# OwshenNetwork/owshen

Hardware: NVIDIA H100
Metric: groth16_withdraw_proofs_per_sec (higher is better)
Workload: dtype u256 (8x32-bit Montgomery limbs, integer)

## Files before the change

owshen_b200/csrc/common.cuh:

```cuda
#pragma once
#include <cuda_runtime.h>
#include <stdint.h>
#include <stdio.h>
#include <string.h>
#include <vector>
#include "../../include/owshen_b200.h"
#include "fp.cuh"
#include "ec.cuh"

namespace og {

constexpr int N_SLOTS = 64;
constexpr int MAX_LANES = 2;

struct NttTables;

}

struct og_ctx {
    int device = 0;
    int sm_count = 132;
    cudaStream_t stream = nullptr;
    cudaStream_t main_stream = nullptr;
    cudaStream_t lane_hi[og::MAX_LANES] = {nullptr}, lane_lo[og::MAX_LANES] = {nullptr};
    cudaEvent_t lane_ev[og::MAX_LANES] = {nullptr}, fork_ev = nullptr;
    cudaStream_t acc_stream = nullptr;
    cudaEvent_t acc_ev = nullptr;
    int lane = 0;
    cudaEvent_t ev0 = nullptr, ev1 = nullptr;
    uint64_t launches = 0;
    char err[512] = {0};
    void* slot_ptr[og::N_SLOTS] = {nullptr};
    size_t slot_cap[og::N_SLOTS] = {0};
    int* d_flag = nullptr;
    int* h_flag = nullptr;
    og::NttTables* ntt[32] = {nullptr};
    void* g1_fixed = nullptr;
    void* g2_fixed = nullptr;
    void* bjj_fixed = nullptr;
    bool digits_smem_opt_in = false;

    bool prof_on = false;
    struct ProfRec { const char* name; cudaEvent_t a, b; };
    std::vector<ProfRec> prof;
    std::vector<cudaEvent_t> ev_pool;
    cudaEvent_t prof_event();

    void* slot(int id, size_t bytes);
};

namespace og {

#define OG_CUDA(ctx, call)                                                                        \
    do {                                                                                          \
        cudaError_t e_ = (call);                                                                  \
        if (e_ != cudaSuccess) {                                                                  \
            snprintf((ctx)->err, sizeof((ctx)->err), "%s:%d: %s: %s", __FILE__, __LINE__, #call,  \
                     cudaGetErrorString(e_));                                                     \
            return OG_E_CUDA;                                                                     \
        }                                                                                         \
    } while (0)

#define OG_TRY(expr)                  \
    do {                              \
        int32_t rc_ = (expr);         \
        if (rc_ != OG_OK) return rc_; \
    } while (0)

#define OG_LAUNCHN(ctx, name, kernel, grid, block, smem, ...)                                     \
    do {                                                                                          \
        cudaEvent_t pa_ = nullptr, pb_ = nullptr;                                                 \
        if ((ctx)->prof_on) { pa_ = (ctx)->prof_event(); pb_ = (ctx)->prof_event();               \
                              cudaEventRecord(pa_, (ctx)->stream); }                              \
        kernel<<<(grid), (block), (smem), (ctx)->stream>>>(__VA_ARGS__);                          \
        if (pa_) { cudaEventRecord(pb_, (ctx)->stream); (ctx)->prof.push_back({(name), pa_, pb_}); } \
        (ctx)->launches++;                                                                        \
        OG_CUDA(ctx, cudaGetLastError());                                                         \
    } while (0)
#define OG_LAUNCH(ctx, kernel, grid, block, smem, ...) OG_LAUNCHN(ctx, #kernel, kernel, grid, block, smem, __VA_ARGS__)

#define OG_SLOT(ctx, var, type, id, bytes)                       \
    type* var = (type*)(ctx)->slot((id), (bytes));               \
    if (!var) return OG_E_NOMEM

enum Slot {
    S_IO_A = 0, S_IO_B, S_IO_C, S_IO_D, S_IO_E, S_IO_F, S_IO_G, S_IO_H,
    S_MSM_POINTS, S_MSM_SCALARS, S_MSM_COUNTS, S_MSM_OFFSETS, S_MSM_CURSOR, S_MSM_SORTED, S_MSM_BUCKETS,
    S_MSM_SEG, S_MSM_OUT, S_MSM_HEAVY, S_MSM_MISC,
    S_NTT_DATA,
    S_PR_WIT, S_PR_ABC, S_PR_SCALARS, S_PR_SORTED, S_PR_COUNTS, S_PR_OFFSETS, S_PR_CURSOR, S_PR_BUCKETS,
    S_PR_SEG, S_PR_SUMS, S_PR_OUT, S_PR_PUB, S_PR_MISC, S_PR_HEAVY,
    S_SETUP_A, S_SETUP_B, S_SETUP_C,
    S_L1_ABC, S_L1_SCALARS, S_L1_SORTED, S_L1_COUNTS, S_L1_OFFSETS, S_L1_CURSOR, S_L1_BUCKETS, S_L1_SEG, S_L1_HEAVY, S_L1_MSM_MISC,
    S_PR_AFF, S_L1_AFF, S_MSM_AFF,
    S_COUNT
};
static_assert(S_COUNT <= N_SLOTS, "grow N_SLOTS");

static inline cudaError_t stream_handoff(cudaEvent_t ev, cudaStream_t from, cudaStream_t to) {
    cudaError_t e = cudaEventRecord(ev, from);
    return e != cudaSuccess ? e : cudaStreamWaitEvent(to, ev, 0);
}

static inline bool aligned32(const void* p) { return (((uintptr_t)p) & 31) == 0; }

int32_t check_flag(og_ctx* ctx);
int32_t clear_flag(og_ctx* ctx);

template <class F>
__device__ __forceinline__ F load_canonical(const uint8_t* p, int* flag) {
    const uint32_t* q = reinterpret_cast<const uint32_t*>(p);
    uint32_t c[8];
#pragma unroll
    for (int i = 0; i < 8; i++) c[i] = q[i];
    if (!F::canonical_lt_mod(c)) { atomicOr(flag, 1); for (int i = 0; i < 8; i++) c[i] = 0; }
    return F::from_canonical(c);
}
template <class F>
__device__ __forceinline__ void store_canonical(uint8_t* p, const F& v) {
    uint32_t c[8];
    v.to_canonical(c);
    uint32_t* q = reinterpret_cast<uint32_t*>(p);
#pragma unroll
    for (int i = 0; i < 8; i++) q[i] = c[i];
}

template <class F>
static inline bool host_load(F& out, const uint8_t* p) {
    uint32_t c[8];
    memcpy(c, p, 32);
    if (!F::canonical_lt_mod(c)) return false;
    out = F::from_canonical(c);
    return true;
}
template <class F>
static inline void host_store(uint8_t* p, const F& v) {
    uint32_t c[8];
    v.to_canonical(c);
    memcpy(p, c, 32);
}

int32_t mimc_init(og_ctx* ctx);
void mimc_constants_host(Fr* out91);

}
```

owshen_b200/csrc/groth16.cu:

```cuda
#include "groth16.cuh"
#include "mimc.cuh"
#include "msm.cuh"
#include "ntt.cuh"
#include "withdraw_circuit.hpp"
#include <stdlib.h>

namespace og {

__global__ void __launch_bounds__(128) k_extras(const uint8_t* __restrict__ rs, uint32_t batch, uint32_t n_vars, uint32_t w_stride,
                                                Fr* __restrict__ W, Fr* __restrict__ rs_m, int* flag) {
    uint32_t p = blockIdx.x * blockDim.x + threadIdx.x;
    if (p >= batch) return;
    Fr r = load_canonical<Fr>(rs + 64ull * p, flag);
    Fr s = load_canonical<Fr>(rs + 64ull * p + 32, flag);
    Fr* w = W + (size_t)p * w_stride;
    w[n_vars] = Fr::one();
    w[n_vars + 1] = r;
    rs_m[2 * p] = r;
    rs_m[2 * p + 1] = s;
}

__global__ void __launch_bounds__(128) k_witness_in(const uint8_t* __restrict__ in, uint32_t batch, uint32_t n_vars, uint32_t w_stride,
                                                    Fr* __restrict__ W, int* flag) {
    uint64_t t = (uint64_t)blockIdx.x * blockDim.x + threadIdx.x;
// ... 220 lines not shown
    memcpy(hC.data() + 64ull * (n_priv + pk->n_supp + m), beta1, 64);

    int32_t rc = OG_OK;
    auto fail = [&](int32_t code) { pk_free(pk); return code; };
    if ((rc = clear_flag(ctx)) != OG_OK) return fail(rc);
    {
        uint8_t* stage;
        if ((rc = upload(ctx, &stage, hA.data(), hA.size())) != OG_OK) return fail(rc);
        if (cudaMalloc(&pk->tabA, sizeof(G1Affine) * (size_t)pk->nA * pk->n_windows[0]) != cudaSuccess) { cudaFree(stage); return fail(OG_E_NOMEM); }
        rc = g1_bytes_to_mont(ctx, stage, pk->nA, pk->tabA);
        if (rc == OG_OK) rc = msm_build_table_g1(ctx, pk->tabA, pk->nA, pk->c[0], pk->n_windows[0]);
        cudaStreamSynchronize(ctx->stream); cudaFree(stage);
        if (rc != OG_OK) return fail(rc);
    }
    {
        uint8_t* stage;
        if ((rc = upload(ctx, &stage, hC.data(), hC.size())) != OG_OK) return fail(rc);
        if (cudaMalloc(&pk->tabC, sizeof(G1Affine) * (size_t)pk->nC * pk->n_windows[2]) != cudaSuccess) { cudaFree(stage); return fail(OG_E_NOMEM); }
        rc = g1_bytes_to_mont(ctx, stage, pk->nC, pk->tabC);
        if (rc == OG_OK) rc = msm_build_table_g1(ctx, pk->tabC, pk->nC, pk->c[2], pk->n_windows[2]);
        cudaStreamSynchronize(ctx->stream); cudaFree(stage);
        if (rc != OG_OK) return fail(rc);
    }
    {
        uint8_t* stage;
        if ((rc = upload(ctx, &stage, hB.data(), hB.size())) != OG_OK) return fail(rc);
        if (cudaMalloc(&pk->tabB, sizeof(G2Affine) * (size_t)pk->nB * pk->n_windows[1]) != cudaSuccess) { cudaFree(stage); return fail(OG_E_NOMEM); }
        rc = g2_bytes_to_mont(ctx, stage, pk->nB, pk->tabB);
        if (rc == OG_OK) rc = msm_build_table_g2(ctx, pk->tabB, pk->nB, pk->c[1], pk->n_windows[1]);
        cudaStreamSynchronize(ctx->stream); cudaFree(stage);
        if (rc != OG_OK) return fail(rc);
    }
    if ((rc = upload(ctx, &pk->supp, supp.data(), 4ull * supp.size())) != OG_OK) return fail(rc);
    cudaStreamSynchronize(ctx->stream);
    if ((rc = upload_csr(ctx, rd, pk->n_constraints, nv, &pk->a_ptr, &pk->a_col, &pk->a_val)) != OG_OK) return fail(rc);
    if ((rc = upload_csr(ctx, rd, pk->n_constraints, nv, &pk->b_ptr, &pk->b_col, &pk->b_val)) != OG_OK) return fail(rc);
    if ((rc = check_flag(ctx)) != OG_OK) return fail(rc);
    *out = pk;
    return OG_OK;
}

bool pk_on_device_of(const og_pk* pk, const og_ctx* ctx) { return pk && ctx && pk->device == ctx->device; }

void pk_info(const og_pk* pk, uint32_t* n_vars, uint32_t* n_pub, uint32_t* log_m, uint32_t* depth) {
    if (n_vars) *n_vars = pk->n_vars;
    if (n_pub) *n_pub = pk->n_pub;
    if (log_m) *log_m = pk->log_m;
    if (depth) *depth = pk->depth;
}

struct ChunkBufs {
    Fr *W, *rs_m, *abc, *ntt_tmp, *bsc, *csc;
    uint32_t *counts, *offsets, *cursor, *sorted, *heavy;
    G1XYZZ *bk1, *lvl1, *totA, *totC;
    G2XYZZ *bk2, *lvl2, *totB;
    void *aff1, *aff2;
    uint32_t w_stride, bsc_stride, csc_stride;
};

#ifdef OG_EXPERIMENT_AFFINE
static uint32_t affine_mode() { return env_u32("OG_AFFINE", 0); }
#else
static uint32_t affine_mode() { return 0; }
#endif

static int32_t alloc_chunk(og_ctx* ctx, const og_pk* pk, uint32_t batch, uint32_t B, int lane, ChunkBufs& b) {
    const uint32_t m = 1u << pk->log_m;
    b.w_stride = pk->n_vars + 2;
    b.bsc_stride = pk->nB;
    b.csc_stride = pk->nC;
    size_t max_pts = pk->nC > pk->nA ? pk->nC : pk->nA;
    size_t n_keys = (size_t)B * pk->max_nb;
    auto S = [&](int id0, int id1) { return lane ? id1 : id0; };
    b.W = (Fr*)ctx->slot(S_PR_WIT, sizeof(Fr) * (size_t)batch * b.w_stride);
    b.rs_m = (Fr*)ctx->slot(S_PR_MISC, sizeof(Fr) * 2 * (size_t)batch);
    b.abc = (Fr*)ctx->slot(S(S_PR_ABC, S_L1_ABC), sizeof(Fr) * (size_t)B * 3 * m * 2);
    b.bsc = (Fr*)ctx->slot(S(S_PR_SCALARS, S_L1_SCALARS), sizeof(Fr) * (size_t)B * (b.bsc_stride + b.csc_stride));
    b.sorted = (uint32_t*)ctx->slot(S(S_PR_SORTED, S_L1_SORTED), 4 * (size_t)B * max_pts * pk->max_windows);
    b.counts = (uint32_t*)ctx->slot(S(S_PR_COUNTS, S_L1_COUNTS), 4 * n_keys);
    b.offsets = (uint32_t*)ctx->slot(S(S_PR_OFFSETS, S_L1_OFFSETS), 4 * (n_keys + 1));
    b.cursor = (uint32_t*)ctx->slot(S(S_PR_CURSOR, S_L1_CURSOR), 4 * n_keys);
    b.heavy = (uint32_t*)ctx->slot(S(S_PR_HEAVY, S_L1_HEAVY), 4 * (2 * n_keys + 4));
    b.bk2 = (G2XYZZ*)ctx->slot(S(S_PR_BUCKETS, S_L1_BUCKETS), sizeof(G2XYZZ) * n_keys);
    b.lvl2 = (G2XYZZ*)ctx->slot(S(S_PR_SEG, S_L1_SEG), sizeof(G2XYZZ) * msm_lvl_elems(B, pk->max_nb));
    b.totA = (G1XYZZ*)ctx->slot(S_PR_SUMS, (sizeof(G1XYZZ) * 2 + sizeof(G2XYZZ)) * (size_t)batch);
    if (!b.W || !b.rs_m || !b.abc || !b.bsc || !b.sorted || !b.counts || !b.offsets || !b.cursor || !b.heavy || !b.bk2 || !b.lvl2 || !b.totA)
        return OG_E_NOMEM;
    b.aff1 = b.aff2 = nullptr;
    if (affine_mode()) {
        size_t need = 0;
        if (affine_mode() & 1) need = msm_aff_scratch_bytes_g1(n_keys);
        if ((affine_mode() & 2) && msm_aff_scratch_bytes_g2((size_t)B * pk->nb[1]) > need) need = msm_aff_scratch_bytes_g2((size_t)B * pk->nb[1]);
        void* a = ctx->slot(S(S_PR_AFF, S_L1_AFF), need);
        if (!a) return OG_E_NOMEM;
        if (affine_mode() & 1) b.aff1 = a;
        if (affine_mode() & 2) b.aff2 = a;
    }
    b.ntt_tmp = b.abc + (size_t)B * 3 * m;
    b.csc = b.bsc + (size_t)B * b.bsc_stride;
    b.bk1 = reinterpret_cast<G1XYZZ*>(b.bk2);
    b.lvl1 = reinterpret_cast<G1XYZZ*>(b.lvl2);
    b.totC = b.totA + batch;
    b.totB = reinterpret_cast<G2XYZZ*>(b.totC + batch);
    return OG_OK;
}

static int32_t run_msm_g1(og_ctx* ctx, const og_pk* pk, int which, ChunkBufs& b, uint32_t B, const G1Affine* table, uint32_t n_pts,
                          const Fr* scalars, uint32_t stride, G1XYZZ* totals) {
    DigitPlan plan;
    plan.scalars = reinterpret_cast<const uint32_t*>(scalars);
    plan.n = n_pts; plan.scalar_stride = stride; plan.n_problems = B;
    plan.c = pk->c[which]; plan.n_windows = pk->n_windows[which]; plan.nb = pk->nb[which];
    plan.key_stride_problem = 1; plan.key_stride_window = 0; plan.tidx_window_stride = n_pts;
    plan.montgomery = 1;
    uint32_t n_keys = B * pk->nb[which];
    OG_TRY(msm_sort_digits(ctx, plan, n_keys, b.counts, b.offsets, b.cursor, b.sorted));
    return msm_buckets_g1(ctx, table, b.sorted, b.offsets, b.counts, B, pk->nb[which], (uint64_t)B * n_pts * pk->n_windows[which], b.bk1, b.lvl1, b.heavy, b.cursor, totals, b.aff1);
}
static int32_t run_msm_g2(og_ctx* ctx, const og_pk* pk, int which, ChunkBufs& b, uint32_t B, const G2Affine* table, uint32_t n_pts,
                          const Fr* scalars, uint32_t stride, G2XYZZ* totals) {
    DigitPlan plan;
    plan.scalars = reinterpret_cast<const uint32_t*>(scalars);
    plan.n = n_pts; plan.scalar_stride = stride; plan.n_problems = B;
    plan.c = pk->c[which]; plan.n_windows = pk->n_windows[which]; plan.nb = pk->nb[which];
    plan.key_stride_problem = 1; plan.key_stride_window = 0; plan.tidx_window_stride = n_pts;
    plan.montgomery = 1;
    uint32_t n_keys = B * pk->nb[which];
    OG_TRY(msm_sort_digits(ctx, plan, n_keys, b.counts, b.offsets, b.cursor, b.sorted));
    return msm_buckets_g2(ctx, table, b.sorted, b.offsets, b.counts, B, pk->nb[which], (uint64_t)B * n_pts * pk->n_windows[which], b.bk2, b.lvl2, b.heavy, b.cursor, totals, b.aff2);
}

struct WitnessSource {
    const uint8_t *d_null = nullptr, *d_sec = nullptr, *d_rec = nullptr, *d_sib = nullptr;
    const uint32_t* d_bits = nullptr;
    const uint8_t* d_wit = nullptr;
    uint8_t* d_public = nullptr;
};

static int32_t prove_chunk(og_ctx* ctx, const og_pk* pk, ChunkBufs& b, const WitnessSource& src, uint32_t off, uint32_t B,
                           const uint8_t* d_rs, uint8_t* d_proofs) {
    const uint32_t m = 1u << pk->log_m, n_priv = pk->n_vars - pk->n_pub - 1;
    Fr* W = b.W + (size_t)off * b.w_stride;
    Fr* rs_m = b.rs_m + 2 * (size_t)off;
    if (src.d_wit) {
        uint64_t tot = (uint64_t)B * pk->n_vars;
        OG_LAUNCH(ctx, k_witness_in, (unsigned)((tot + 127) / 128), 128, 0, src.d_wit + 32ull * off * pk->n_vars, B, pk->n_vars, b.w_stride, W, ctx->d_flag);
    } else {
        WithdrawLayout L = WithdrawLayout::make(pk->depth);
        OG_TRY(withdraw_witness_strided_dev(ctx, L, b.w_stride, src.d_null + 32ull * off, src.d_sec + 32ull * off, src.d_rec + 32ull * off,
                                            src.d_sib + 32ull * off * pk->depth, src.d_bits + off, B, W));
        if (src.d_public) OG_LAUNCH(ctx, k_public_out, (B * pk->n_pub + 127) / 128, 128, 0, W, b.w_stride, B, pk->n_pub, src.d_public + 32ull * off * pk->n_pub);
    }
    OG_LAUNCH(ctx, k_extras, (B + 127) / 128, 128, 0, d_rs + 64ull * off, B, pk->n_vars, b.w_stride, W, rs_m, ctx->d_flag);
    CsrDev A{pk->a_ptr, pk->a_col, pk->a_val}, Bm{pk->b_ptr, pk->b_col, pk->b_val};
    OG_LAUNCH(ctx, k_abc, dim3((m + 127) / 128, B), 128, 0, A, Bm, pk->n_constraints, pk->n_pub, pk->log_m, W, b.w_stride, B, b.abc);
    OG_TRY(ntt_mont_dev(ctx, b.abc, b.ntt_tmp, pk->log_m, 3 * B, 1, 0, 1));
    OG_TRY(ntt_mont_dev(ctx, b.abc, b.ntt_tmp, pk->log_m, 3 * B, 0, 1, 2));
    uint32_t mx = n_priv > pk->n_supp ? n_priv : pk->n_supp;
    OG_LAUNCH(ctx, k_compose, dim3((mx + 127) / 128, B), 128, 0, W, b.w_stride, rs_m, pk->supp, pk->n_supp, pk->n_vars, pk->n_pub, m,
              b.bsc, b.bsc_stride, b.csc, b.csc_stride);
    OG_LAUNCH(ctx, k_pointwise, dim3((m + 127) / 128, B), 128, 0, b.abc, pk->log_m, B, b.csc, b.csc_stride, n_priv + pk->n_supp);
    OG_TRY(run_msm_g1(ctx, pk, 0, b, B, pk->tabA, pk->nA, W, b.w_stride, b.totA + off));
    OG_TRY(run_msm_g1(ctx, pk, 2, b, B, pk->tabC, pk->nC, b.csc, b.csc_stride, b.totC + off));
    OG_TRY(run_msm_g2(ctx, pk, 1, b, B, pk->tabB, pk->nB, b.bsc, b.bsc_stride, b.totB + off));
    OG_LAUNCH(ctx, k_assemble_g1, (B + 31) / 32, 32, 0, b.totA + off, b.totC + off, rs_m, B, d_proofs + 256ull * off);
    OG_LAUNCH(ctx, k_assemble_g2, (B + 31) / 32, 32, 0, b.totB + off, B, d_proofs + 256ull * off);
    return OG_OK;
}

static uint32_t chunk_limit(const og_pk* pk) {
    uint64_t max_pts = pk->nC > pk->nA ? pk->nC : pk->nA;
    uint64_t by_entries = 0xF0000000ull / (max_pts * pk->max_windows);
    uint64_t by_keys = 0x7FFFFFFFull / pk->max_nb;
    uint64_t lim = by_entries < by_keys ? by_entries : by_keys;
    return (uint32_t)(lim < 1 ? 1 : lim);
}

static uint32_t chunk_size(const og_pk* pk, uint32_t batch) {
    uint32_t c = env_u32("OG_CHUNK", 1024);
    if (c > chunk_limit(pk)) c = chunk_limit(pk);
    return c < batch ? c : batch;
// ... 77 lines not shown
```

owshen_b200/csrc/msm.cu:

```cuda
#include "msm.cuh"
#include "glv.cuh"
#include <stdlib.h>
#if !defined(OG_MSM_G1) && !defined(OG_MSM_G2)
#error "compile msm.cu with -DOG_MSM_G1 or -DOG_MSM_G2"
#endif

namespace og {

template <class F> struct FieldIO;
template <> struct FieldIO<Fq> {
    static constexpr int BYTES = 32;
    static __device__ __forceinline__ Fq load(const uint8_t* p, int* flag) { return load_canonical<Fq>(p, flag); }
    static __device__ __forceinline__ void store(uint8_t* p, const Fq& v) { store_canonical(p, v); }
};
template <> struct FieldIO<Fq2> {
    static constexpr int BYTES = 64;
    static __device__ __forceinline__ Fq2 load(const uint8_t* p, int* flag) {
        return Fq2{load_canonical<Fq>(p, flag), load_canonical<Fq>(p + 32, flag)};
    }
    static __device__ __forceinline__ void store(uint8_t* p, const Fq2& v) { store_canonical(p, v.c0); store_canonical(p + 32, v.c1); }
};

template <class F>
__global__ void __launch_bounds__(128) k_points_to_mont(const uint8_t* __restrict__ in, uint64_t n, Affine<F>* __restrict__ out, int* flag) {
// ... 10 lines not shown
    constexpr int B = FieldIO<F>::BYTES;
    Affine<F> p = in[i];
    FieldIO<F>::store(out + 2 * B * i, p.x);
    FieldIO<F>::store(out + 2 * B * i + B, p.y);
}

#ifdef OG_MSM_G1
int32_t g1_bytes_to_mont(og_ctx* ctx, const uint8_t* d_in, uint64_t n, G1Affine* d_out) {
    if (n) OG_LAUNCH(ctx, k_points_to_mont<Fq>, (unsigned)((n + 127) / 128), 128, 0, d_in, n, d_out, ctx->d_flag);
    return OG_OK;
}
#endif

#ifdef OG_MSM_G2
int32_t g2_bytes_to_mont(og_ctx* ctx, const uint8_t* d_in, uint64_t n, G2Affine* d_out) {
    if (n) OG_LAUNCH(ctx, k_points_to_mont<Fq2>, (unsigned)((n + 127) / 128), 128, 0, d_in, n, d_out, ctx->d_flag);
    return OG_OK;
}
#endif

#ifdef OG_MSM_G1
int32_t g1_mont_to_bytes(og_ctx* ctx, const G1Affine* d_in, uint64_t n, uint8_t* d_out) {
    if (n) OG_LAUNCH(ctx, k_points_from_mont<Fq>, (unsigned)((n + 127) / 128), 128, 0, d_in, n, d_out);
    return OG_OK;
}
#endif

#ifdef OG_MSM_G2
int32_t g2_mont_to_bytes(og_ctx* ctx, const G2Affine* d_in, uint64_t n, uint8_t* d_out) {
    if (n) OG_LAUNCH(ctx, k_points_from_mont<Fq2>, (unsigned)((n + 127) / 128), 128, 0, d_in, n, d_out);
    return OG_OK;
}
#endif


#ifdef OG_MSM_G1
struct DigitIter {
    uint32_t s[9];
    __device__ __forceinline__ bool load(const DigitPlan& P, uint32_t prob, uint64_t i, int* flag) {
        const uint32_t* sp = P.scalars + ((uint64_t)prob * P.scalar_stride + i) * 8;
        if (P.montgomery) {
            Fr v;
#pragma unroll
            for (int j = 0; j < 8; j++) v.l[j] = sp[j];
            v.to_canonical(s);
        } else {
#pragma unroll
            for (int j = 0; j < 8; j++) s[j] = sp[j];
            if (!Fr::canonical_lt_mod(s)) { atomicOr(flag, 1); return false; }
        }
        s[8] = 0;
        return (s[0] | s[1] | s[2] | s[3] | s[4] | s[5] | s[6] | s[7]) != 0;
    }
    template <class Fn>
    __device__ __forceinline__ void for_each(const DigitPlan& P, Fn f) const {
        const uint32_t c = P.c, half = 1u << (c - 1), mask = (1u << c) - 1;
        uint32_t carry = 0;
        for (uint32_t w = 0; w < P.n_windows; w++) {
            uint32_t bit = w * c, word = bit >> 5, sh = bit & 31;
            uint64_t two = ((uint64_t)s[word + 1] << 32) | s[word];
            uint32_t v = ((uint32_t)(two >> sh) & mask) + carry;
            uint32_t neg = v > half;
            uint32_t mag = neg ? (1u << c) - v : v;
            carry = neg;
            if (mag) f(w, mag - 1, neg);
        }
    }
};

template <bool SCATTER>
__global__ void __launch_bounds__(256) k_digits(DigitPlan P, uint32_t* __restrict__ counts, const uint32_t* __restrict__ offsets,
                                                uint32_t* __restrict__ cursor, uint32_t* __restrict__ sorted, int* flag) {
    uint64_t i = (uint64_t)blockIdx.x * blockDim.x + threadIdx.x;
    uint32_t prob = blockIdx.y;
    if (i >= P.n) return;
    DigitIter it;
    if (!it.load(P, prob, i, flag)) return;
    it.for_each(P, [&](uint32_t w, uint32_t b, uint32_t neg) {
        uint32_t key = (prob * P.key_stride_problem + w * P.key_stride_window) * P.nb + b;
        if (!SCATTER) {
            atomicAdd(&counts[key], 1u);
        } else {
            uint32_t pos = atomicAdd(&cursor[key], 1u);
            sorted[pos] = (((uint32_t)i + w * P.tidx_window_stride) << 1) | neg;
        }
    });
}

constexpr uint32_t DIG_TILE = 4096, DIG_THREADS = 256, DIG_MAX_NB_COUNT = 32768;

__global__ void __launch_bounds__(DIG_THREADS) k_digits_count_tiled(DigitPlan P, uint32_t* __restrict__ counts, int* flag) {
    extern __shared__ uint32_t hist[];
    const uint32_t prob = blockIdx.y, nb = P.nb;
    const uint64_t lo = (uint64_t)blockIdx.x * DIG_TILE;
    const uint64_t hi = lo + DIG_TILE < P.n ? lo + DIG_TILE : P.n;
    const uint32_t key0 = prob * P.key_stride_problem * nb;
    for (uint32_t b = threadIdx.x; b < nb; b += DIG_THREADS) hist[b] = 0;
    __syncthreads();
    for (uint64_t i = lo + threadIdx.x; i < hi; i += DIG_THREADS) {
        DigitIter it;
        if (it.load(P, prob, i, flag)) it.for_each(P, [&](uint32_t, uint32_t b, uint32_t) { atomicAdd(&hist[b], 1u); });
    }
    __syncthreads();
    for (uint32_t b = threadIdx.x; b < nb; b += DIG_THREADS) if (hist[b]) atomicAdd(&counts[key0 + b], hist[b]);
}

constexpr uint32_t SCAN_THREADS = 256, SCAN_PER_THREAD = 8, SCAN_TILE = SCAN_THREADS * SCAN_PER_THREAD;

__device__ __forceinline__ uint32_t block_exclusive_scan(uint32_t v, uint32_t* total) {
    __shared__ uint32_t warp_sums[SCAN_THREADS / 32];
    __shared__ uint32_t block_total;
    uint32_t lane = threadIdx.x & 31, wid = threadIdx.x >> 5;
    uint32_t inc = v;
#pragma unroll
    for (int d = 1; d < 32; d <<= 1) { uint32_t t = __shfl_up_sync(0xffffffffu, inc, d); if (lane >= (uint32_t)d) inc += t; }
    if (lane == 31) warp_sums[wid] = inc;
    __syncthreads();
    if (wid == 0) {
        uint32_t w = lane < SCAN_THREADS / 32 ? warp_sums[lane] : 0, winc = w;
#pragma unroll
        for (int d = 1; d < 8; d <<= 1) { uint32_t t = __shfl_up_sync(0xffffffffu, winc, d); if (lane >= (uint32_t)d) winc += t; }
        if (lane < SCAN_THREADS / 32) warp_sums[lane] = winc - w;
        if (lane == SCAN_THREADS / 32 - 1) block_total = winc;
    }
    __syncthreads();
    uint32_t r = inc - v + warp_sums[wid];
    *total = block_total;
    __syncthreads();
    return r;
}

__global__ void __launch_bounds__(SCAN_THREADS) k_scan_tiles(const uint32_t* __restrict__ counts, uint32_t n, uint32_t* __restrict__ tile_sums) {
    uint32_t base = blockIdx.x * SCAN_TILE + threadIdx.x * SCAN_PER_THREAD, s = 0;
#pragma unroll
    for (uint32_t k = 0; k < SCAN_PER_THREAD; k++) if (base + k < n) s += counts[base + k];
    uint32_t total;
    block_exclusive_scan(s, &total);
    if (threadIdx.x == 0) tile_sums[blockIdx.x] = total;
}
__global__ void __launch_bounds__(SCAN_THREADS) k_scan_tile_sums(uint32_t* __restrict__ tile_sums, uint32_t n_tiles, uint32_t* __restrict__ grand_total) {
    uint32_t run = 0;
    for (uint32_t base = 0; base < n_tiles; base += SCAN_THREADS) {
        uint32_t i = base + threadIdx.x;
        uint32_t v = i < n_tiles ? tile_sums[i] : 0, total;
        uint32_t ex = block_exclusive_scan(v, &total);
        if (i < n_tiles) tile_sums[i] = run + ex;
        run += total;
    }
    if (threadIdx.x == 0) *grand_total = run;
}
__global__ void __launch_bounds__(SCAN_THREADS) k_scan_apply(const uint32_t* __restrict__ counts, uint32_t n, const uint32_t* __restrict__ tile_sums,
                                                            uint32_t* __restrict__ offsets, uint32_t* __restrict__ cursor) {
    uint32_t base = blockIdx.x * SCAN_TILE + threadIdx.x * SCAN_PER_THREAD;
    uint32_t c[SCAN_PER_THREAD], s = 0;
#pragma unroll
    for (uint32_t k = 0; k < SCAN_PER_THREAD; k++) { c[k] = base + k < n ? counts[base + k] : 0; s += c[k]; }
    uint32_t total;
    uint32_t run = tile_sums[blockIdx.x] + block_exclusive_scan(s, &total);
#pragma unroll
    for (uint32_t k = 0; k < SCAN_PER_THREAD; k++) {
        if (base + k < n) { offsets[base + k] = run; cursor[base + k] = run; }
        run += c[k];
    }
}

int32_t msm_sort_digits(og_ctx* ctx, const DigitPlan& plan, uint32_t n_keys, uint32_t* d_counts, uint32_t* d_offsets,
                        uint32_t* d_cursor, uint32_t* d_sorted) {
    OG_CUDA(ctx, cudaMemsetAsync(d_counts, 0, sizeof(uint32_t) * (size_t)n_keys, ctx->stream));
    if (plan.n == 0 || plan.n_problems == 0) {
        OG_CUDA(ctx, cudaMemsetAsync(d_offsets, 0, sizeof(uint32_t) * ((size_t)n_keys + 1), ctx->stream));
        return OG_OK;
    }
    const bool tiled = plan.key_stride_window == 0 && plan.nb <= DIG_MAX_NB_COUNT;
    if (tiled && !ctx->digits_smem_opt_in) {
        OG_CUDA(ctx, cudaFuncSetAttribute(k_digits_count_tiled, cudaFuncAttributeMaxDynamicSharedMemorySize, (int)(4 * DIG_MAX_NB_COUNT)));
        ctx->digits_smem_opt_in = true;
    }
    dim3 grid((unsigned)((plan.n + 255) / 256), plan.n_problems);
    dim3 tgrid((unsigned)((plan.n + DIG_TILE - 1) / DIG_TILE), plan.n_problems);
    if (tiled) OG_LAUNCH(ctx, k_digits_count_tiled, tgrid, DIG_THREADS, 4 * (size_t)plan.nb, plan, d_counts, ctx->d_flag);
    else OG_LAUNCHN(ctx, "k_digits_count", k_digits<false>, grid, 256, 0, plan, d_counts, nullptr, nullptr, nullptr, ctx->d_flag);
    {
        uint32_t n_tiles = (n_keys + SCAN_TILE - 1) / SCAN_TILE;
        OG_SLOT(ctx, tile_sums, uint32_t, ctx->lane ? S_L1_MSM_MISC : S_MSM_MISC, 4 * (size_t)n_tiles);
        OG_LAUNCH(ctx, k_scan_tiles, n_tiles, SCAN_THREADS, 0, d_counts, n_keys, tile_sums);
        OG_LAUNCH(ctx, k_scan_tile_sums, 1, SCAN_THREADS, 0, tile_sums, n_tiles, d_offsets + n_keys);
        OG_LAUNCH(ctx, k_scan_apply, n_tiles, SCAN_THREADS, 0, d_counts, n_keys, tile_sums, d_offsets, d_cursor);
    }
    OG_LAUNCHN(ctx, "k_digits_scatter", k_digits<true>, grid, 256, 0, plan, d_counts, d_offsets, d_cursor, d_sorted, ctx->d_flag);
    return OG_OK;
}
#endif


constexpr uint32_t ORDER_BINS = 2048;
template <class F>
__global__ void __launch_bounds__(1024) k_bucket_order(const uint32_t* __restrict__ counts, uint32_t nb, uint32_t* __restrict__ perm) {
    __shared__ uint32_t hist[ORDER_BINS];
    const uint32_t g = blockIdx.x, t = threadIdx.x;
    const uint32_t* c = counts + (size_t)g * nb;
    for (uint32_t i = t; i < ORDER_BINS; i += 1024) hist[i] = 0;
    __syncthreads();
    for (uint32_t b = t; b < nb; b += 1024) atomicAdd(&hist[ORDER_BINS - 1 - min(c[b], ORDER_BINS - 1)], 1u);
    __syncthreads();
    __shared__ uint32_t pair[1024];
    uint32_t a0 = hist[2 * t], a1 = hist[2 * t + 1];
    pair[t] = a0 + a1;
    __syncthreads();
    for (uint32_t d = 1; d < 1024; d <<= 1) {
        uint32_t v = t >= d ? pair[t - d] : 0;
        __syncthreads();
        pair[t] += v;
        __syncthreads();
    }
    uint32_t base = t ? pair[t - 1] : 0;
    hist[2 * t] = base;
    hist[2 * t + 1] = base + a0;
    __syncthreads();
    for (uint32_t b = t; b < nb; b += 1024) {
        uint32_t pos = atomicAdd(&hist[ORDER_BINS - 1 - min(c[b], ORDER_BINS - 1)], 1u);
        perm[(size_t)g * nb + pos] = g * nb + b;
    }
}

template <class F>
__device__ __forceinline__ Affine<F> fetch_point(const Affine<F>* __restrict__ table, uint32_t e) {
    Affine<F> p = table[e >> 1];
    if (e & 1) p.y = p.y.neg();
    return p;
}

#ifdef OG_MSM_G1
struct SmAcc1 {
    uint4* base;
    __device__ __forceinline__ Fq ld(int coord) const {
        Fq v;
        uint4 a = base[(coord * 2 + 0) * 128], b = base[(coord * 2 + 1) * 128];
        v.l[0] = a.x; v.l[1] = a.y; v.l[2] = a.z; v.l[3] = a.w; v.l[4] = b.x; v.l[5] = b.y; v.l[6] = b.z; v.l[7] = b.w;
        return v;
    }
    __device__ __forceinline__ void st(int coord, const Fq& v) const {
// ... 818 lines not shown
```

owshen_b200/csrc/msm.cuh:

```cuda
#pragma once
#include "common.cuh"

namespace og {

struct DigitPlan {
    const uint32_t* scalars;
    uint64_t n;
    uint64_t scalar_stride;
    uint32_t n_problems;
    uint32_t c, n_windows, nb;
    uint32_t key_stride_problem, key_stride_window;
    uint32_t tidx_window_stride;
    int32_t montgomery;
};

static inline uint32_t msm_windows(uint32_t c) { return (255 + c - 1) / c; }

int32_t msm_sort_digits(og_ctx* ctx, const DigitPlan& plan, uint32_t n_keys, uint32_t* d_counts,
                        uint32_t* d_offsets , uint32_t* d_cursor, uint32_t* d_sorted);

int32_t msm_buckets_g1(og_ctx* ctx, const G1Affine* d_table, const uint32_t* d_sorted, const uint32_t* d_offsets,
                       const uint32_t* d_counts, uint32_t n_groups, uint32_t nb, uint64_t n_entries_max, G1XYZZ* d_buckets,
                       G1XYZZ* d_lvl, uint32_t* d_heavy, uint32_t* d_perm, G1XYZZ* d_totals, void* aff_scratch = nullptr);
int32_t msm_buckets_g2(og_ctx* ctx, const G2Affine* d_table, const uint32_t* d_sorted, const uint32_t* d_offsets,
                       const uint32_t* d_counts, uint32_t n_groups, uint32_t nb, uint64_t n_entries_max, G2XYZZ* d_buckets,
                       G2XYZZ* d_lvl, uint32_t* d_heavy, uint32_t* d_perm, G2XYZZ* d_totals, void* aff_scratch = nullptr);
size_t msm_aff_scratch_bytes_g1(uint64_t n_keys);
size_t msm_aff_scratch_bytes_g2(uint64_t n_keys);
static inline size_t msm_lvl_elems(uint32_t n_groups, uint32_t nb) { return 4 * ((size_t)n_groups * ((nb + 7) / 8) + 16); }

int32_t msm_g1_dev(og_ctx* ctx, const uint8_t* d_points, const uint8_t* d_scalars, uint64_t n, uint8_t* d_out64);
int32_t msm_g2_dev(og_ctx* ctx, const uint8_t* d_points, const uint8_t* d_scalars, uint64_t n, uint8_t* d_out128);
int32_t sum_g1_dev(og_ctx* ctx, const uint8_t* d_points, uint64_t n, uint8_t* d_out64);
int32_t sum_g2_dev(og_ctx* ctx, const uint8_t* d_points, uint64_t n, uint8_t* d_out128);

int32_t g1_bytes_to_mont(og_ctx* ctx, const uint8_t* d_in, uint64_t n, G1Affine* d_out);
int32_t g2_bytes_to_mont(og_ctx* ctx, const uint8_t* d_in, uint64_t n, G2Affine* d_out);
int32_t g1_mont_to_bytes(og_ctx* ctx, const G1Affine* d_in, uint64_t n, uint8_t* d_out);
int32_t g2_mont_to_bytes(og_ctx* ctx, const G2Affine* d_in, uint64_t n, uint8_t* d_out);

int32_t msm_build_table_g1(og_ctx* ctx, G1Affine* d_table, uint32_t n, uint32_t c, uint32_t n_windows);
int32_t msm_build_table_g2(og_ctx* ctx, G2Affine* d_table, uint32_t n, uint32_t c, uint32_t n_windows);

int32_t fixed_base_mul_g1(og_ctx* ctx, const uint8_t* d_scalars, uint64_t n, G1Affine* d_out);
int32_t fixed_base_mul_g2(og_ctx* ctx, const uint8_t* d_scalars, uint64_t n, G2Affine* d_out);

}
```

Measured before the change: 1889.

## Replace atomic digit scatter with two-level partitioned bucket sort for MSM

Replaces the MSM digit sort (a global histogram, a scan, then atomic scatter into every bucket) with a two-level sort when windows share keys. Each tile first counts scalar digits into up to 128 coarse partitions using warp-aggregated shared-memory atomics, and the per-tile counts are scanned. A scatter kernel then writes staged entries in rounds through shared memory, and a per-partition local kernel sorts by fine bucket and writes counts, offsets and sorted indices. The aim is to cut scattered global atomics and uncoalesced writes. The cost is extra staging buffers, which reuse the bucket and heavy memory when they fit, and more kernel launches. Other callers that do not supply staging buffers now get an invalid-argument error on this path.

New measurement: 2013 (median of 6 runs). 6.6% higher.

```diff
diff --git a/owshen_b200/csrc/common.cuh b/owshen_b200/csrc/common.cuh
--- a/owshen_b200/csrc/common.cuh
+++ b/owshen_b200/csrc/common.cuh
@@ -38,7 +38,6 @@
     void* g1_fixed = nullptr;
     void* g2_fixed = nullptr;
     void* bjj_fixed = nullptr;
-    bool digits_smem_opt_in = false;
 
     bool prof_on = false;
     struct ProfRec { const char* name; cudaEvent_t a, b; };
@@ -93,6 +92,7 @@
     S_SETUP_A, S_SETUP_B, S_SETUP_C,
     S_L1_ABC, S_L1_SCALARS, S_L1_SORTED, S_L1_COUNTS, S_L1_OFFSETS, S_L1_CURSOR, S_L1_BUCKETS, S_L1_SEG, S_L1_HEAVY, S_L1_MSM_MISC,
     S_PR_AFF, S_L1_AFF, S_MSM_AFF,
+    S_PR_SORT_STAGE, S_L1_SORT_STAGE, S_PR_SORT_TILES, S_L1_SORT_TILES,
     S_COUNT
 };
 static_assert(S_COUNT <= N_SLOTS, "grow N_SLOTS");
diff --git a/owshen_b200/csrc/groth16.cu b/owshen_b200/csrc/groth16.cu
--- a/owshen_b200/csrc/groth16.cu
+++ b/owshen_b200/csrc/groth16.cu
@@ -296,6 +296,7 @@
 struct ChunkBufs {
     Fr *W, *rs_m, *abc, *ntt_tmp, *bsc, *csc;
     uint32_t *counts, *offsets, *cursor, *sorted, *heavy;
+    uint32_t *sort_stage, *sort_tiles;
     G1XYZZ *bk1, *lvl1, *totA, *totC;
     G2XYZZ *bk2, *lvl2, *totB;
     void *aff1, *aff2;
@@ -342,6 +343,12 @@
     }
     b.ntt_tmp = b.abc + (size_t)B * 3 * m;
     b.csc = b.bsc + (size_t)B * b.bsc_stride;
+    const uint32_t n_pts[3] = {pk->nA, pk->nB, pk->nC};
+    size_t stage = msm_sort_stage_bytes((size_t)B * max_pts * pk->max_windows), tiles = 0;
+    for (int k = 0; k < 3; k++) { size_t t = msm_sort_tile_bytes(B, pk->nb[k], n_pts[k]); if (t > tiles) tiles = t; }
+    b.sort_stage = stage <= sizeof(G2XYZZ) * n_keys ? (uint32_t*)b.bk2 : (uint32_t*)ctx->slot(S(S_PR_SORT_STAGE, S_L1_SORT_STAGE), stage);
+    b.sort_tiles = tiles <= 4 * (2 * n_keys + 4) ? b.heavy : (uint32_t*)ctx->slot(S(S_PR_SORT_TILES, S_L1_SORT_TILES), tiles);
+    if (!b.sort_stage || !b.sort_tiles) return OG_E_NOMEM;
     b.bk1 = reinterpret_cast<G1XYZZ*>(b.bk2);
     b.lvl1 = reinterpret_cast<G1XYZZ*>(b.lvl2);
     b.totC = b.totA + batch;
@@ -358,7 +365,7 @@
     plan.key_stride_problem = 1; plan.key_stride_window = 0; plan.tidx_window_stride = n_pts;
     plan.montgomery = 1;
     uint32_t n_keys = B * pk->nb[which];
-    OG_TRY(msm_sort_digits(ctx, plan, n_keys, b.counts, b.offsets, b.cursor, b.sorted));
+    OG_TRY(msm_sort_digits(ctx, plan, n_keys, b.counts, b.offsets, nullptr, b.sorted, b.sort_stage, b.sort_tiles));
     return msm_buckets_g1(ctx, table, b.sorted, b.offsets, b.counts, B, pk->nb[which], (uint64_t)B * n_pts * pk->n_windows[which], b.bk1, b.lvl1, b.heavy, b.cursor, totals, b.aff1);
 }
 static int32_t run_msm_g2(og_ctx* ctx, const og_pk* pk, int which, ChunkBufs& b, uint32_t B, const G2Affine* table, uint32_t n_pts,
@@ -370,7 +377,7 @@
     plan.key_stride_problem = 1; plan.key_stride_window = 0; plan.tidx_window_stride = n_pts;
     plan.montgomery = 1;
     uint32_t n_keys = B * pk->nb[which];
-    OG_TRY(msm_sort_digits(ctx, plan, n_keys, b.counts, b.offsets, b.cursor, b.sorted));
+    OG_TRY(msm_sort_digits(ctx, plan, n_keys, b.counts, b.offsets, nullptr, b.sorted, b.sort_stage, b.sort_tiles));
     return msm_buckets_g2(ctx, table, b.sorted, b.offsets, b.counts, B, pk->nb[which], (uint64_t)B * n_pts * pk->n_windows[which], b.bk2, b.lvl2, b.heavy, b.cursor, totals, b.aff2);
 }
 
diff --git a/owshen_b200/csrc/msm.cu b/owshen_b200/csrc/msm.cu
--- a/owshen_b200/csrc/msm.cu
+++ b/owshen_b200/csrc/msm.cu
@@ -86,8 +86,31 @@
         s[8] = 0;
         return (s[0] | s[1] | s[2] | s[3] | s[4] | s[5] | s[6] | s[7]) != 0;
     }
+    __device__ __forceinline__ void clear() {
+#pragma unroll
+        for (int j = 0; j < 9; j++) s[j] = 0;
+    }
+    static __device__ __forceinline__ void fetch(const DigitPlan& P, uint32_t prob, uint64_t i, uint32_t raw[8]) {
+        const uint4* sp = reinterpret_cast<const uint4*>(P.scalars + ((uint64_t)prob * P.scalar_stride + i) * 8);
+        const uint4 a = sp[0], b = sp[1];
+        raw[0] = a.x; raw[1] = a.y; raw[2] = a.z; raw[3] = a.w; raw[4] = b.x; raw[5] = b.y; raw[6] = b.z; raw[7] = b.w;
+    }
+    __device__ __forceinline__ bool from_raw(const DigitPlan& P, const uint32_t raw[8], int* flag) {
+        if (P.montgomery) {
+            Fr v;
+#pragma unroll
+            for (int j = 0; j < 8; j++) v.l[j] = raw[j];
+            v.to_canonical(s);
+        } else {
+#pragma unroll
+            for (int j = 0; j < 8; j++) s[j] = raw[j];
+            if (!Fr::canonical_lt_mod(s)) { atomicOr(flag, 1); return false; }
+        }
+        s[8] = 0;
+        return (s[0] | s[1] | s[2] | s[3] | s[4] | s[5] | s[6] | s[7]) != 0;
+    }
     template <class Fn>
-    __device__ __forceinline__ void for_each(const DigitPlan& P, Fn f) const {
+    __device__ __forceinline__ void windows(const DigitPlan& P, Fn f) const {
         const uint32_t c = P.c, half = 1u << (c - 1), mask = (1u << c) - 1;
         uint32_t carry = 0;
         for (uint32_t w = 0; w < P.n_windows; w++) {
@@ -97,8 +120,12 @@
             uint32_t neg = v > half;
             uint32_t mag = neg ? (1u << c) - v : v;
             carry = neg;
-            if (mag) f(w, mag - 1, neg);
-        }
+            f(w, mag, neg);
+        }
+    }
+    template <class Fn>
+    __device__ __forceinline__ void for_each(const DigitPlan& P, Fn f) const {
+        windows(P, [&](uint32_t w, uint32_t mag, uint32_t neg) { if (mag) f(w, mag - 1, neg); });
     }
 };
 
@@ -121,24 +148,6 @@
     });
 }
 
-constexpr uint32_t DIG_TILE = 4096, DIG_THREADS = 256, DIG_MAX_NB_COUNT = 32768;
-
-__global__ void __launch_bounds__(DIG_THREADS) k_digits_count_tiled(DigitPlan P, uint32_t* __restrict__ counts, int* flag) {
-    extern __shared__ uint32_t hist[];
-    const uint32_t prob = blockIdx.y, nb = P.nb;
-    const uint64_t lo = (uint64_t)blockIdx.x * DIG_TILE;
-    const uint64_t hi = lo + DIG_TILE < P.n ? lo + DIG_TILE : P.n;
-    const uint32_t key0 = prob * P.key_stride_problem * nb;
-    for (uint32_t b = threadIdx.x; b < nb; b += DIG_THREADS) hist[b] = 0;
-    __syncthreads();
-    for (uint64_t i = lo + threadIdx.x; i < hi; i += DIG_THREADS) {
-        DigitIter it;
-        if (it.load(P, prob, i, flag)) it.for_each(P, [&](uint32_t, uint32_t b, uint32_t) { atomicAdd(&hist[b], 1u); });
-    }
-    __syncthreads();
-    for (uint32_t b = threadIdx.x; b < nb; b += DIG_THREADS) if (hist[b]) atomicAdd(&counts[key0 + b], hist[b]);
-}
-
 constexpr uint32_t SCAN_THREADS = 256, SCAN_PER_THREAD = 8, SCAN_TILE = SCAN_THREADS * SCAN_PER_THREAD;
 
 __device__ __forceinline__ uint32_t block_exclusive_scan(uint32_t v, uint32_t* total) {
@@ -193,34 +202,186 @@
     uint32_t run = tile_sums[blockIdx.x] + block_exclusive_scan(s, &total);
 #pragma unroll
     for (uint32_t k = 0; k < SCAN_PER_THREAD; k++) {
-        if (base + k < n) { offsets[base + k] = run; cursor[base + k] = run; }
+        if (base + k < n) { offsets[base + k] = run; if (cursor) cursor[base + k] = run; }
         run += c[k];
     }
 }
 
+static int32_t exclusive_scan(og_ctx* ctx, const uint32_t* d_counts, uint32_t n, uint32_t* d_offsets, uint32_t* d_cursor) {
+    uint32_t n_tiles = (n + SCAN_TILE - 1) / SCAN_TILE;
+    OG_SLOT(ctx, tile_sums, uint32_t, ctx->lane ? S_L1_MSM_MISC : S_MSM_MISC, 4 * (size_t)n_tiles);
+    OG_LAUNCH(ctx, k_scan_tiles, n_tiles, SCAN_THREADS, 0, d_counts, n, tile_sums);
+    OG_LAUNCH(ctx, k_scan_tile_sums, 1, SCAN_THREADS, 0, tile_sums, n_tiles, d_offsets + n);
+    OG_LAUNCH(ctx, k_scan_apply, n_tiles, SCAN_THREADS, 0, d_counts, n, tile_sums, d_offsets, d_cursor);
+    return OG_OK;
+}
+
+constexpr uint32_t SORT_PARTS = 128, SORT_TILE = 4096, SORT_THREADS = 256;
+constexpr uint32_t SORT_MAX_NB = 32768, SORT_MAX_FINE = SORT_MAX_NB / SORT_PARTS;
+constexpr uint32_t NO_BIN = 0xFFFFFFFFu;
+static_assert(SORT_THREADS == SCAN_THREADS, "k_sort_local scans with block_exclusive_scan");
+static_assert(SORT_PARTS <= SORT_THREADS && SORT_MAX_FINE <= SORT_THREADS && SORT_TILE % SORT_THREADS == 0, "sort shape");
+static_assert(SORT_MAX_FINE <= 256, "fine bucket ids are staged as one byte");
+
+static uint32_t sort_parts(uint32_t nb) { return nb < SORT_PARTS ? nb : SORT_PARTS; }
+static uint32_t sort_shift(uint32_t nb) { uint32_t s = 0; while ((sort_parts(nb) << s) < nb) s++; return s; }
+static uint64_t sort_tiles(uint64_t n) { return (n + SORT_TILE - 1) / SORT_TILE; }
+
+__device__ __forceinline__ uint32_t warp_bin_add(uint32_t* bins, uint32_t bin) {
+    const uint32_t lane = threadIdx.x & 31, valid = __ballot_sync(0xffffffffu, bin != NO_BIN);
+    if (!valid) return 0;
+    const uint32_t leader = __ffs(valid) - 1, first = __shfl_sync(0xffffffffu, bin, leader);
+    if (__all_sync(0xffffffffu, bin == NO_BIN || bin == first)) {
+        uint32_t base = 0;
+        if (lane == leader) base = atomicAdd(&bins[first], (uint32_t)__popc(valid));
+        return __shfl_sync(0xffffffffu, base, leader) + __popc(valid & ((1u << lane) - 1));
+    }
+    return bin != NO_BIN ? atomicAdd(&bins[bin], 1u) : 0;
+}
+
+__global__ void __launch_bounds__(SORT_THREADS) k_sort_part_count(DigitPlan P, uint32_t shift, uint32_t n_tiles,
+                                                                  uint32_t* __restrict__ tile_counts, int* flag) {
+    __shared__ uint32_t hist[SORT_PARTS];
+    const uint32_t prob = blockIdx.y, tile = blockIdx.x, parts = P.nb >> shift;
+    for (uint32_t p = threadIdx.x; p < parts; p += SORT_THREADS) hist[p] = 0;
+    __syncthreads();
+    const uint64_t lo = (uint64_t)tile * SORT_TILE, hi = lo + SORT_TILE < P.n ? lo + SORT_TILE : P.n;
+    uint32_t raw[8];
+    if (lo + threadIdx.x < hi) DigitIter::fetch(P, prob, lo + threadIdx.x, raw);
+    for (uint64_t i0 = lo; i0 < hi; i0 += SORT_THREADS) {
+        const uint64_t i = i0 + threadIdx.x;
+        DigitIter it;
+        if (!(i < hi && it.from_raw(P, raw, flag))) it.clear();
+        if (i + SORT_THREADS < hi) DigitIter::fetch(P, prob, i + SORT_THREADS, raw);
+        it.windows(P, [&](uint32_t, uint32_t mag, uint32_t) { warp_bin_add(hist, mag ? (mag - 1) >> shift : NO_BIN); });
+    }
+    __syncthreads();
+    for (uint32_t p = threadIdx.x; p < parts; p += SORT_THREADS) tile_counts[((size_t)prob * parts + p) * n_tiles + tile] = hist[p];
+}
+
+constexpr uint32_t SORT_ROUND_WINDOWS = 24, SORT_ROUND = SORT_THREADS * SORT_ROUND_WINDOWS;
+__global__ void __launch_bounds__(SORT_THREADS) k_sort_part_scatter(DigitPlan P, uint32_t shift, uint32_t n_tiles,
+                                                                    const uint32_t* __restrict__ tile_offs, uint32_t* __restrict__ stage_e,
+                                                                    uint8_t* __restrict__ stage_f, int* flag) {
+    __shared__ uint32_t sm_e[SORT_ROUND];
+    __shared__ uint16_t sm_b[SORT_ROUND];
+    __shared__ uint32_t cnt[SORT_PARTS], lbase[SORT_PARTS], cur[SORT_PARTS];
+    const uint32_t tid = threadIdx.x, prob = blockIdx.y, tile = blockIdx.x, parts = P.nb >> shift, fmask = (1u << shift) - 1;
+    for (uint32_t p = tid; p < parts; p += SORT_THREADS) { cur[p] = tile_offs[((size_t)prob * parts + p) * n_tiles + tile]; cnt[p] = 0; }
+    __syncthreads();
+    const uint64_t lo = (uint64_t)tile * SORT_TILE, hi = lo + SORT_TILE < P.n ? lo + SORT_TILE : P.n;
+    uint32_t raw[8];
+    if (lo + tid < hi) DigitIter::fetch(P, prob, lo + tid, raw);
+    for (uint64_t i0 = lo; i0 < hi; i0 += SORT_THREADS) {
+        const uint64_t i = i0 + tid;
+        DigitIter it;
+        if (!(i < hi && it.from_raw(P, raw, flag))) it.clear();
+        if (i + SORT_THREADS < hi) DigitIter::fetch(P, prob, i + SORT_THREADS, raw);
+        for (uint32_t w0 = 0; w0 < P.n_windows; w0 += SORT_ROUND_WINDOWS) {
+            auto bin_of = [&](uint32_t w, uint32_t mag) { return mag && w >= w0 && w < w0 + SORT_ROUND_WINDOWS ? (mag - 1) >> shift : NO_BIN; };
+            it.windows(P, [&](uint32_t w, uint32_t mag, uint32_t) { warp_bin_add(cnt, bin_of(w, mag)); });
+            __syncthreads();
+            uint32_t n_round, b = block_exclusive_scan(tid < parts ? cnt[tid] : 0, &n_round);
+            if (tid < parts) { lbase[tid] = b; cnt[tid] = b; }
+            __syncthreads();
+            it.windows(P, [&](uint32_t w, uint32_t mag, uint32_t neg) {
+                const uint32_t bin = bin_of(w, mag), pos = warp_bin_add(cnt, bin);
+                if (bin != NO_BIN) { sm_e[pos] = (((uint32_t)i + w * P.tidx_window_stride) << 1) | neg; sm_b[pos] = (uint16_t)(mag - 1); }
+            });
+            __syncthreads();
+            for (uint32_t k = tid; k < n_round; k += SORT_THREADS) {
+                const uint32_t bk = sm_b[k], p = bk >> shift, dst = cur[p] + k - lbase[p];
+                stage_e[dst] = sm_e[k];
+                stage_f[dst] = (uint8_t)(bk & fmask);
+            }
+            __syncthreads();
+            if (tid < parts) { cur[tid] += cnt[tid] - lbase[tid]; cnt[tid] = 0; }
+            __syncthreads();
+        }
+    }
+}
+
+constexpr uint32_t SORT_LOCAL_CAP = 10240;
+constexpr uint32_t SORT_LOCAL_ITEMS = 8, SORT_LOCAL_STEP = SORT_THREADS * SORT_LOCAL_ITEMS;
+__global__ void __launch_bounds__(SORT_THREADS) k_sort_local(const uint32_t* __restrict__ tile_offs, uint32_t n_tiles, uint32_t n_parts,
+                                                             uint32_t shift, const uint32_t* __restrict__ total,
+                                                             const uint32_t* __restrict__ stage_e, const uint8_t* __restrict__ stage_f,
+                                                             uint32_t* __restrict__ counts, uint32_t* __restrict__ offsets,
+                                                             uint32_t* __restrict__ sorted) {
+    __shared__ uint32_t bins[SORT_THREADS];
+    __shared__ uint32_t sm_out[SORT_LOCAL_CAP];
+    const uint32_t g = blockIdx.x, F = 1u << shift, tid = threadIdx.x;
+    const uint32_t start = tile_offs[(size_t)g * n_tiles], end = g + 1 < n_parts ? tile_offs[(size_t)(g + 1) * n_tiles] : *total;
+    if (g + 1 == n_parts && tid == 0) offsets[(size_t)n_parts * F] = end;
+    bins[tid] = 0;
+    __syncthreads();
+    for (uint32_t j0 = start; j0 < end; j0 += SORT_LOCAL_STEP) {
+        uint32_t f[SORT_LOCAL_ITEMS];
+#pragma unroll
+        for (uint32_t k = 0; k < SORT_LOCAL_ITEMS; k++) { const uint32_t j = j0 + k * SORT_THREADS + tid; f[k] = j < end ? stage_f[j] : NO_BIN; }
+#pragma unroll
+        for (uint32_t k = 0; k < SORT_LOCAL_ITEMS; k++) warp_bin_add(bins, f[k]);
+    }
+    __syncthreads();
+    const uint32_t c = tid < F ? bins[tid] : 0;
+    uint32_t tot;
+    const uint32_t run = start + block_exclusive_scan(c, &tot);
+    if (tid < F) {
+        const size_t key = (size_t)g * F + tid;
+        counts[key] = c; offsets[key] = run; bins[tid] = run;
+    }
+    __syncthreads();
+    const bool staged = end - start <= SORT_LOCAL_CAP;
+    for (uint32_t j0 = start; j0 < end; j0 += SORT_LOCAL_STEP) {
+        uint32_t f[SORT_LOCAL_ITEMS], e[SORT_LOCAL_ITEMS];
+#pragma unroll
+        for (uint32_t k = 0; k < SORT_LOCAL_ITEMS; k++) {
+            const uint32_t j = j0 + k * SORT_THREADS + tid;
+            f[k] = j < end ? stage_f[j] : NO_BIN;
+            e[k] = j < end ? stage_e[j] : 0;
+        }
+#pragma unroll
+        for (uint32_t k = 0; k < SORT_LOCAL_ITEMS; k++) {
+            const uint32_t pos = warp_bin_add(bins, f[k]);
+            if (f[k] != NO_BIN) { if (staged) sm_out[pos - start] = e[k]; else sorted[pos] = e[k]; }
+        }
+    }
+    if (staged) {
+        __syncthreads();
+        for (uint32_t k = tid; k < end - start; k += SORT_THREADS) sorted[start + k] = sm_out[k];
+    }
+}
+
+size_t msm_sort_stage_bytes(uint64_t n_entries) { return 5 * n_entries; }
+size_t msm_sort_tile_bytes(uint32_t n_problems, uint32_t nb, uint64_t n) { return 8 * (size_t)n_problems * sort_parts(nb) * sort_tiles(n) + 4; }
+
 int32_t msm_sort_digits(og_ctx* ctx, const DigitPlan& plan, uint32_t n_keys, uint32_t* d_counts, uint32_t* d_offsets,
-                        uint32_t* d_cursor, uint32_t* d_sorted) {
-    OG_CUDA(ctx, cudaMemsetAsync(d_counts, 0, sizeof(uint32_t) * (size_t)n_keys, ctx->stream));
+                        uint32_t* d_cursor, uint32_t* d_sorted, uint32_t* d_stage, uint32_t* d_tiles) {
     if (plan.n == 0 || plan.n_problems == 0) {
+        OG_CUDA(ctx, cudaMemsetAsync(d_counts, 0, sizeof(uint32_t) * (size_t)n_keys, ctx->stream));
         OG_CUDA(ctx, cudaMemsetAsync(d_offsets, 0, sizeof(uint32_t) * ((size_t)n_keys + 1), ctx->stream));
         return OG_OK;
     }
-    const bool tiled = plan.key_stride_window == 0 && plan.nb <= DIG_MAX_NB_COUNT;
-    if (tiled && !ctx->digits_smem_opt_in) {
-        OG_CUDA(ctx, cudaFuncSetAttribute(k_digits_count_tiled, cudaFuncAttributeMaxDynamicSharedMemorySize, (int)(4 * DIG_MAX_NB_COUNT)));
-        ctx->digits_smem_opt_in = true;
-    }
+    if (plan.key_stride_window == 0) {
+        if (!d_stage || !d_tiles || plan.key_stride_problem != 1 || plan.nb > SORT_MAX_NB || n_keys != plan.n_problems * plan.nb) return OG_E_INVALID;
+        const uint32_t parts = sort_parts(plan.nb), shift = sort_shift(plan.nb), n_tiles = (uint32_t)sort_tiles(plan.n);
+        const uint32_t n_parts = plan.n_problems * parts, n_runs = n_parts * n_tiles;
+        uint32_t* tile_counts = d_tiles;
+        uint32_t* tile_offs = d_tiles + n_runs;
+        uint32_t* stage_e = d_stage;
+        uint8_t* stage_f = reinterpret_cast<uint8_t*>(d_stage + (uint64_t)plan.n_problems * plan.n * plan.n_windows);
+        dim3 tgrid(n_tiles, plan.n_problems);
+        OG_LAUNCH(ctx, k_sort_part_count, tgrid, SORT_THREADS, 0, plan, shift, n_tiles, tile_counts, ctx->d_flag);
+        OG_TRY(exclusive_scan(ctx, tile_counts, n_runs, tile_offs, nullptr));
+        OG_LAUNCH(ctx, k_sort_part_scatter, tgrid, SORT_THREADS, 0, plan, shift, n_tiles, tile_offs, stage_e, stage_f, ctx->d_flag);
+        OG_LAUNCH(ctx, k_sort_local, n_parts, SORT_THREADS, 0, tile_offs, n_tiles, n_parts, shift, tile_offs + n_runs, stage_e, stage_f,
+                  d_counts, d_offsets, d_sorted);
+        return OG_OK;
+    }
+    OG_CUDA(ctx, cudaMemsetAsync(d_counts, 0, sizeof(uint32_t) * (size_t)n_keys, ctx->stream));
     dim3 grid((unsigned)((plan.n + 255) / 256), plan.n_problems);
-    dim3 tgrid((unsigned)((plan.n + DIG_TILE - 1) / DIG_TILE), plan.n_problems);
-    if (tiled) OG_LAUNCH(ctx, k_digits_count_tiled, tgrid, DIG_THREADS, 4 * (size_t)plan.nb, plan, d_counts, ctx->d_flag);
-    else OG_LAUNCHN(ctx, "k_digits_count", k_digits<false>, grid, 256, 0, plan, d_counts, nullptr, nullptr, nullptr, ctx->d_flag);
-    {
-        uint32_t n_tiles = (n_keys + SCAN_TILE - 1) / SCAN_TILE;
-        OG_SLOT(ctx, tile_sums, uint32_t, ctx->lane ? S_L1_MSM_MISC : S_MSM_MISC, 4 * (size_t)n_tiles);
-        OG_LAUNCH(ctx, k_scan_tiles, n_tiles, SCAN_THREADS, 0, d_counts, n_keys, tile_sums);
-        OG_LAUNCH(ctx, k_scan_tile_sums, 1, SCAN_THREADS, 0, tile_sums, n_tiles, d_offsets + n_keys);
-        OG_LAUNCH(ctx, k_scan_apply, n_tiles, SCAN_THREADS, 0, d_counts, n_keys, tile_sums, d_offsets, d_cursor);
-    }
+    OG_LAUNCHN(ctx, "k_digits_count", k_digits<false>, grid, 256, 0, plan, d_counts, nullptr, nullptr, nullptr, ctx->d_flag);
+    OG_TRY(exclusive_scan(ctx, d_counts, n_keys, d_offsets, d_cursor));
     OG_LAUNCHN(ctx, "k_digits_scatter", k_digits<true>, grid, 256, 0, plan, d_counts, d_offsets, d_cursor, d_sorted, ctx->d_flag);
     return OG_OK;
 }
diff --git a/owshen_b200/csrc/msm.cuh b/owshen_b200/csrc/msm.cuh
--- a/owshen_b200/csrc/msm.cuh
+++ b/owshen_b200/csrc/msm.cuh
@@ -17,7 +17,10 @@
 static inline uint32_t msm_windows(uint32_t c) { return (255 + c - 1) / c; }
 
 int32_t msm_sort_digits(og_ctx* ctx, const DigitPlan& plan, uint32_t n_keys, uint32_t* d_counts,
-                        uint32_t* d_offsets , uint32_t* d_cursor, uint32_t* d_sorted);
+                        uint32_t* d_offsets , uint32_t* d_cursor, uint32_t* d_sorted,
+                        uint32_t* d_stage = nullptr, uint32_t* d_tiles = nullptr);
+size_t msm_sort_stage_bytes(uint64_t n_entries);
+size_t msm_sort_tile_bytes(uint32_t n_problems, uint32_t nb, uint64_t n);
 
 int32_t msm_buckets_g1(og_ctx* ctx, const G1Affine* d_table, const uint32_t* d_sorted, const uint32_t* d_offsets,
                        const uint32_t* d_counts, uint32_t n_groups, uint32_t nb, uint64_t n_entries_max, G1XYZZ* d_buckets,
```
